# sp-uhh/audio-visual-vad

Hardware: AMD Instinct MI355X
Metric: AV frame-pairs/sec (fwd+bwd) (higher is better)
Workload: dtype f32; 1 GPU; AV_net fused training step (WaveNet-W0 encoder + ResNet-18 trunk + concat + 2xLSTM1024 + FC, masked BCE, backward, RCCL all-reduce, fused Adam): BASELINE configs[3]/[4] per-GPU shard; per_gpu_frame_pairs=1024, global_frame_pairs=1024, sequences_per_gpu=64, parallelism=dp1, reserved_cus=0, reported_block=median

## Files before the change

audio-visual-vad_amd/csrc/wavenet.hip:

```cpp
#include "gemm_api.h"
#include "wn_block.h"
#include "wn_tail.h"

namespace {

static inline int grid1(long n) { long b = (n + 255) / 256; return (int)(b > 8192 ? 8192 : (b < 1 ? 1 : b)); }

__global__ void conv1d_fwd_generic(const float* __restrict__ x, const float* __restrict__ w, const float* __restrict__ bias,
                                   const float* __restrict__ res, float* __restrict__ y, int B, int Cin, int Cout, int Lin,
                                   int Lout, int fw, int dil, int relu_in, int res_off, int res_L) {
  const long n = (long)B * Cout * Lout;
  for (long i = (long)blockIdx.x * blockDim.x + threadIdx.x; i < n; i += (long)gridDim.x * blockDim.x) {
    const int t = (int)(i % Lout);
    const int co = (int)((i / Lout) % Cout);
    const int b = (int)(i / ((long)Lout * Cout));
    float acc = bias ? bias[co] : 0.f;
    const float* xb = x + (long)b * Cin * Lin + t;
    const float* wr = w + (long)co * Cin * fw;
    for (int ci = 0; ci < Cin; ++ci)
      for (int k = 0; k < fw; ++k) {
        float v = xb[(long)ci * Lin + k * dil];
        if (relu_in) v = fmaxf(v, 0.f);
        acc = fmaf(wr[ci * fw + k], v, acc);
      }
// ... 635 lines not shown

struct DzwTile { float g[16], x[32]; };
template <bool RESIDENT>
__device__ __forceinline__ void wn_block_bwd_dz_wgrad_body(float* tiles, float* red, float* wl, float* wtl,
                                                           const float* __restrict__ dS, const float* __restrict__ w_dil,
                                                           const float* __restrict__ b_dil, const float* __restrict__ w_dense,
                                                           const float* __restrict__ s_in, float* __restrict__ DZ,
                                                           float* __restrict__ slab, int B, int Lin, int dil) {
  const int lane = threadIdx.x & 63, wave = threadIdx.x >> 6;
  const int li = lane & 31, lh = lane >> 5;
  const int Lo = Lin - dil;
  const int tiles_per_seq = tiles_per_sequence<32>(Lo);
  const int ntiles = B * tiles_per_seq;
  float* T = tiles + wave * 2 * 1056;
  float* T1 = T + 1056;
  float* Th = T + lh * 1056;
  stage_w_dil(wl, w_dil, threadIdx.x, 256);
  stage_bias(wl + WIMG_DIL_SIZE, b_dil, threadIdx.x);
  if (RESIDENT) stage_w_dense(T, w_dense, lane, 64);
  else stage_w_dense(wtl, w_dense, threadIdx.x, 256);
  for (int i = threadIdx.x; i < WG_SLAB; i += 256) red[i] = 0.f;
  __syncthreads();
  const float* wtp = (RESIDENT ? T : wtl) + lh * WIMG_DENSE_PITCH + li;
  const float* wdp = wl + li * WIMG_DIL_PITCH + lh;
  const float* bzl = wl + WIMG_DIL_SIZE + 4 * lh;
  float wt[16], wd[32];
  if (RESIDENT) {
#pragma unroll
    for (int s = 0; s < 16; ++s) wt[s] = wtp[2 * WIMG_DENSE_PITCH * s];
#pragma unroll
    for (int s = 0; s < 32; ++s) wd[s] = wdp[2 * s];
  }
  __builtin_amdgcn_wave_barrier();

  f32x16 acc0, acc1, acc2;
#pragma unroll
  for (int r = 0; r < 16; ++r) { acc0[r] = 0.f; acc1[r] = 0.f; acc2[r] = 0.f; }
  float bs_dz = 0.f, bs_ds = 0.f;
  const int rowL = Lin * 4, rowO = Lo * 4;

  auto issue = [&](int tile, DzwTile& n) __attribute__((always_inline)) {
    const TilePos p = tile_pos(tile < ntiles ? tile : ntiles - 1, tiles_per_seq, li, Lo);
    const __amdgpu_buffer_rsrc_t rg = brsrc(dS + (long)p.b * 32 * Lo, 32 * rowO);
    const __amdgpu_buffer_rsrc_t rx = brsrc(s_in + (long)p.b * 32 * Lin, 32 * rowL);
    const int offg = p.ok ? p.t * 4 + lh * rowO : BUF_OOB;
    const int offx = p.ok ? (p.t + lh * dil) * 4 : BUF_OOB;
#pragma unroll
    for (int q = 0; q < 16; ++q) n.g[q] = bload(rg, offg, 2 * q * rowO);
#pragma unroll
    for (int c = 0; c < 32; ++c) n.x[c] = bload(rx, offx, c * rowL);
  };
  auto compute = [&](int tidx, const DzwTile& c) __attribute__((always_inline)) {
    const TilePos p = tile_pos(tidx, tiles_per_seq, li, Lo);
    const int offo = p.ok ? p.t * 4 + 4 * lh * rowO : BUF_OOB;
    const __amdgpu_buffer_rsrc_t rz = brsrc(DZ + (long)p.b * 32 * Lo, 32 * rowO);
    float x[32];
#pragma unroll
    for (int s = 0; s < 32; ++s) x[s] = relu1(c.x[s]);
    f32x16 z;
#pragma unroll
    for (int r = 0; r < 16; ++r) z[r] = bzl[mfma32_row(r, 0)];
#pragma unroll
    for (int s = 0; s < 32; ++s) z = mfma32(RESIDENT ? wd[s] : wdp[2 * s], x[s], z);
    f32x16 acc;
#pragma unroll
    for (int r = 0; r < 16; ++r) acc[r] = 0.f;
#pragma unroll
    for (int q = 0; q < 16; ++q) acc = mfma32(RESIDENT ? wt[q] : wtp[2 * WIMG_DENSE_PITCH * q], c.g[q], acc);
    float f0[16], f1[16];
    __builtin_amdgcn_wave_barrier();
#pragma unroll
    for (int r = 0; r < 16; ++r) {
      const float dz = z[r] > 0.f ? acc[r] : 0.f;
      bstore(dz, rz, offo, mfma32_row(r, 0) * rowO);
      T[mfma32_row(r, lh) * 33 + li] = dz;
    }
    __builtin_amdgcn_wave_barrier();
#pragma unroll
    for (int q = 0; q < 16; ++q) { f0[q] = T[li * 33 + 2 * q + lh]; bs_dz += f0[q]; }
    __builtin_amdgcn_wave_barrier();
#pragma unroll
    for (int s = 0; s < 32; ++s) Th[s * 33 + li] = x[s];
    __builtin_amdgcn_wave_barrier();
#pragma unroll
    for (int q = 0; q < 16; ++q) f1[q] = T[li * 33 + 2 * q + lh];
#pragma unroll
    for (int q = 0; q < 16; ++q) acc0 = mfma32(f0[q], f1[q], acc0);
#pragma unroll
    for (int q = 0; q < 16; ++q) f1[q] = T1[li * 33 + 2 * q + lh];
#pragma unroll
    for (int q = 0; q < 16; ++q) acc1 = mfma32(f0[q], f1[q], acc1);
    __builtin_amdgcn_wave_barrier();
#pragma unroll
    for (int q = 0; q < 16; ++q) T[(2 * q + lh) * 33 + li] = c.g[q];
#pragma unroll
    for (int r = 0; r < 16; ++r) T1[mfma32_row(r, lh) * 33 + li] = relu1(z[r]);
    __builtin_amdgcn_wave_barrier();
#pragma unroll
    for (int q = 0; q < 16; ++q) { f0[q] = T[li * 33 + 2 * q + lh]; bs_ds += f0[q]; }
#pragma unroll
    for (int q = 0; q < 16; ++q) f1[q] = T1[li * 33 + 2 * q + lh];
#pragma unroll
    for (int q = 0; q < 16; ++q) acc2 = mfma32(f0[q], f1[q], acc2);
    __builtin_amdgcn_wave_barrier();
  };
  const TileWalkI w = xcd_walk_i(ntiles);
  DzwTile ta, tb;
  if (RESIDENT) {
    if (w.first < w.last) issue(w.first, ta);
    pingpong_tiles<true>(w, ta, tb, issue, compute);
  } else {
    plain_tiles<true, DzwTile>(w, issue, compute);
  }

  for (int wv = 0; wv < 4; ++wv) {
    __syncthreads();
    if (wave == wv) {
#pragma unroll
      for (int r = 0; r < 16; ++r) {
        const int row = mfma32_row(r, lh);
        red[row * 32 + li] += acc0[r];
        red[1024 + row * 32 + li] += acc1[r];
        red[2048 + row * 32 + li] += acc2[r];
      }
      if (lh == 0) { red[3072 + li] += bs_dz; red[3104 + li] += bs_ds; }
      __builtin_amdgcn_wave_barrier();
      if (lh == 1) { red[3072 + li] += bs_dz; red[3104 + li] += bs_ds; }
    }
  }
  __syncthreads();
  float* out = slab + (long)blockIdx.x * WG_SLAB;
  for (int i = threadIdx.x; i < WG_SLAB; i += 256) out[i] = red[i];
}

__global__ void __launch_bounds__(256)
    wn_block_bwd_dz_wgrad_mfma(const float* __restrict__ dS, const float* __restrict__ w_dil, const float* __restrict__ b_dil,
                               const float* __restrict__ w_dense, const float* __restrict__ s_in, float* __restrict__ DZ,
                               float* __restrict__ slab, int B, int Lin, int dil) {
  __shared__ float tile[4 * 2 * 32 * 33];
  __shared__ float red[WG_SLAB];
  __shared__ float wl[WIMG_DIL_SIZE + 32];
  wn_block_bwd_dz_wgrad_body<true>(tile, red, wl, nullptr, dS, w_dil, b_dil, w_dense, s_in, DZ, slab, B, Lin, dil);
}

__global__ void __launch_bounds__(256, 2)
    wn_block_bwd_dz_wgrad_occ(const float* __restrict__ dS, const float* __restrict__ w_dil, const float* __restrict__ b_dil,
                               const float* __restrict__ w_dense, const float* __restrict__ s_in, float* __restrict__ DZ,
                               float* __restrict__ slab, int B, int Lin, int dil) {
  __shared__ float tile[4 * 2 * 32 * 33];
  __shared__ float red[WG_SLAB];
  __shared__ float wl[WIMG_DIL_SIZE + 32];
  __shared__ float wtl[WIMG_DENSE_SIZE];
  wn_block_bwd_dz_wgrad_body<false>(tile, red, wl, wtl, dS, w_dil, b_dil, w_dense, s_in, DZ, slab, B, Lin, dil);
}

typedef float f4u __attribute__((ext_vector_type(4), aligned(4)));

__global__ void __launch_bounds__(256, 2)
    wn_block_bwd_dzw_t(const float* __restrict__ dS, const float* __restrict__ w_dil, const float* __restrict__ b_dil,
                       const float* __restrict__ w_dense, const float* __restrict__ s_in, float* __restrict__ DZ,
                       float* __restrict__ slab, int B, int Lin, int dil) {
  __shared__ float red[WG_SLAB];
  __shared__ float wl[WIMG_BDENSE];
  const int lane = threadIdx.x & 63;
  const int li = lane & 31, lh = lane >> 5;
  const int Lo = Lin - dil;
  const int tiles_per_seq = tiles_per_sequence<32>(Lo);
  const long ntiles = (long)B * tiles_per_seq;
  const long wave0 = ((long)blockIdx.x * blockDim.x + threadIdx.x) >> 6;
  const long nwaves = ((long)gridDim.x * blockDim.x) >> 6;
  stage_w_dil(wl + WIMG_DIL, w_dil, threadIdx.x, 256);
  stage_w_dense(wl + WIMG_DENSE, w_dense, threadIdx.x, 256);
  stage_bias(wl + WIMG_BDIL, b_dil, threadIdx.x);
  for (int i = threadIdx.x; i < WG_SLAB; i += 256) red[i] = 0.f;
  __syncthreads();
  const float* wdp = wl + WIMG_DIL + li * WIMG_DIL_PITCH + lh;
  const float* wtp = wl + WIMG_DENSE + lh * WIMG_DENSE_PITCH + li;
  const float bz = wl[WIMG_BDIL + li];

  f32x16 acc0, acc1, acc2;
#pragma unroll
  for (int r = 0; r < 16; ++r) { acc0[r] = 0.f; acc1[r] = 0.f; acc2[r] = 0.f; }
  float bs_dz = 0.f, bs_ds = 0.f;

  for (long tl = wave0; tl < ntiles; tl += nwaves) {
    const TilePos p = tile_pos(tl, tiles_per_seq, li, Lo);
    const int b = p.b, t0 = p.t0, t = p.t;
    const bool ok = p.ok;
    const int tcl = ok ? t : 0;
    const bool full = t0 + 32 <= Lo;
    float x[32], g[16];
    {
      const float* xp = s_in + (long)b * 32 * Lin + tcl + lh * dil;
#pragma unroll
      for (int c = 0; c < 32; ++c) x[c] = xp[(long)c * Lin];
      const float* gp = dS + (long)b * 32 * Lo + tcl;
#pragma unroll
      for (int q = 0; q < 16; ++q) g[q] = gp[(long)(2 * q + lh) * Lo];
    }
    float gc[16], xc0[16], xc1[16];
    const float* rowS = dS + ((long)b * 32 + li) * Lo + t0 + 4 * lh;
    const float* rowX = s_in + ((long)b * 32 + li) * Lin + t0 + 4 * lh;
    if (full) {
#pragma unroll
      for (int q = 0; q < 4; ++q) {
        const f4u a = *reinterpret_cast<const f4u*>(rowS + 8 * q);
        const f4u u = *reinterpret_cast<const f4u*>(rowX + 8 * q);
        const f4u v = *reinterpret_cast<const f4u*>(rowX + dil + 8 * q);
#pragma unroll
        for (int e = 0; e < 4; ++e) { gc[4 * q + e] = a[e]; xc0[4 * q + e] = u[e]; xc1[4 * q + e] = v[e]; }
      }
    } else {
#pragma unroll
      for (int s = 0; s < 16; ++s) {
        const int o = 8 * (s >> 2) + (s & 3);
        const bool in = t0 + 4 * lh + o < Lo;
        const int oc = in ? o : -(t0 + 4 * lh);
        const float a = rowS[oc], u = rowX[oc], v = rowX[oc + dil];
        gc[s] = in ? a : 0.f; xc0[s] = in ? u : 0.f; xc1[s] = in ? v : 0.f;
      }
    }
    __builtin_amdgcn_sched_barrier(0);
#pragma unroll
    for (int c = 0; c < 32; ++c) x[c] = ok ? relu1(x[c]) : 0.f;
#pragma unroll
    for (int q = 0; q < 16; ++q) g[q] = ok ? g[q] : 0.f;
    f32x16 zT;
#pragma unroll
    for (int r = 0; r < 16; ++r) zT[r] = bz;
#pragma unroll
    for (int s = 0; s < 32; ++s) zT = mfma32(x[s], wdp[2 * s], zT);
    f32x16 dzT;
#pragma unroll
    for (int r = 0; r < 16; ++r) dzT[r] = 0.f;
#pragma unroll
    for (int s = 0; s < 16; ++s) dzT = mfma32(g[s], wtp[66 * s], dzT);
#pragma unroll
    for (int r = 0; r < 16; ++r) dzT[r] = zT[r] > 0.f ? dzT[r] : 0.f;
    float* rowZ = DZ + ((long)b * 32 + li) * Lo + t0 + 4 * lh;
    if (full) {
#pragma unroll
      for (int q = 0; q < 4; ++q) {
        f4u o = {dzT[4 * q], dzT[4 * q + 1], dzT[4 * q + 2], dzT[4 * q + 3]};
        *reinterpret_cast<f4u*>(rowZ + 8 * q) = o;
      }
    } else {
#pragma unroll
      for (int s = 0; s < 16; ++s) {
        const int o = 8 * (s >> 2) + (s & 3);
        if (t0 + 4 * lh + o < Lo) rowZ[o] = dzT[s];
      }
    }
#pragma unroll
    for (int s = 0; s < 16; ++s) { bs_dz += dzT[s]; bs_ds += gc[s]; }
#pragma unroll
    for (int s = 0; s < 16; ++s) acc2 = mfma32(gc[s], relu1(zT[s]), acc2);
#pragma unroll
    for (int s = 0; s < 16; ++s) acc0 = mfma32(dzT[s], relu1(xc0[s]), acc0);
#pragma unroll
    for (int s = 0; s < 16; ++s) acc1 = mfma32(dzT[s], relu1(xc1[s]), acc1);
  }

#pragma unroll
  for (int r = 0; r < 16; ++r) {
    const int row = mfma32_row(r, lh);
    atomicAdd(&red[row * 32 + li], acc0[r]);
    atomicAdd(&red[1024 + row * 32 + li], acc1[r]);
    atomicAdd(&red[2048 + row * 32 + li], acc2[r]);
  }
  atomicAdd(&red[3072 + li], bs_dz);
  atomicAdd(&red[3104 + li], bs_ds);
  __syncthreads();
  float* out = slab + (long)blockIdx.x * WG_SLAB;
  for (int i = threadIdx.x; i < WG_SLAB; i += 256) out[i] = red[i];
}

constexpr int WN_MAXL = 64;
struct WgradTab {
  const float* slab[WN_MAXL];
  int nslab[WN_MAXL];
  float* dW_dil[WN_MAXL];
  float* db_dil[WN_MAXL];
  float* dW_dense[WN_MAXL];
  float* db_dense[WN_MAXL];
};
__global__ void __launch_bounds__(256) wn_wgrad_reduce_all(const WgradTab tab) {
  const int l = blockIdx.y;
  const int i = blockIdx.x * 32 + (threadIdx.x & 31);
  const int nslab = tab.nslab[l];
  const float s = slab_sum_fixed_order(tab.slab[l] + i, nslab, WG_SLAB);
  if (threadIdx.x >= 32 || nslab <= 0) return;
  if (i < 2048) { if (tab.dW_dil[l]) tab.dW_dil[l][(i & 1023) * 2 + (i >> 10)] += s; }
  else if (i < 3072) { if (tab.dW_dense[l]) tab.dW_dense[l][i - 2048] += s; }
  else if (i < 3104) { if (tab.db_dil[l]) tab.db_dil[l][i - 3072] += s; }
  else if (tab.db_dense[l]) tab.db_dense[l][i - 3104] += s;
}

struct Plan {
  int n;
  int L[66];
  size_t s[66];
  size_t z, dz, ga, gb, dzt;
  size_t zs[66];
  size_t slab;
  size_t gslab;
  size_t total;
};
static int make_plan(const avvad_wavenet_desc* d, Plan* p) {
  if (!d || d->n_layers < 0 || d->n_layers > 64 || d->B <= 0 || d->fw < 1 || d->qc < 1 || d->R < 1 || d->D < 1 ||
      d->Bn < 1 || d->P < 1 || (d->n_layers > 0 && !d->dilations_h))
    return AVVAD_EINVAL;
  p->n = d->n_layers;
  p->L[0] = d->L - (d->fw - 1);
  for (int i = 0; i < p->n; ++i) p->L[i + 1] = p->L[i] - d->dilations_h[i] * (d->fw - 1);
  if (p->L[p->n] < 1) return AVVAD_EINVAL;
  size_t off = 0;
  auto take = [&](size_t n) { size_t o = off; off += align_up(n, 64); return o; };
  const size_t B = d->B;
  if (d->save_for_backward) {
    for (int i = 0; i <= p->n; ++i) p->s[i] = take(B * d->R * p->L[i]);
    const size_t big = B * (size_t)(d->R > d->D ? d->R : d->D) * p->L[0];
    p->z = take(big); p->dz = take(big); p->ga = take(big); p->gb = take(big);
    p->dzt = take(B * d->Bn * p->L[p->n]);
    {
      const size_t zb = (d->R == 32 && d->D == 32 && d->fw == 2 && p->n > 0) ? take(B * d->D * p->L[1]) : 0;
      for (int i = 0; i < p->n; ++i) p->zs[i] = zb;
    }
    {
      const bool perlayer = d->R == 32 && d->D == 32 && d->fw == 2;
      const size_t a = (size_t)WG_MAXBLK * WG_SLAB * (perlayer ? (size_t)p->n : 1), b2 = (size_t)TAIL_MAXBLK * tail_slab_floats(d->Bn);
      p->slab = take(a > b2 ? a : b2);
    }
    p->gslab = take(igemm::SLAB_FLOATS);
  } else {
    for (int i = 0; i < p->n; ++i) p->zs[i] = 0;
    const size_t a = take(B * d->R * p->L[0]), b2 = take(B * d->R * p->L[0]);
    for (int i = 0; i <= p->n; ++i) p->s[i] = (i & 1) ? b2 : a;
    p->z = take(B * d->D * p->L[0]);
    p->dz = p->ga = p->gb = p->dzt = 0;
  }
  p->total = off;
  return AVVAD_OK;
}

static inline bool mfma_shape(const avvad_wavenet_desc* d) { return d->R == 32 && d->D == 32 && d->fw == 2; }
static inline bool buf_ok(int B, int Lin) {
  return avvad_tune().wn_flat != 1 && (long)Lin * 32 * 4 + 4096 < (1L << 31) && (long)B * cdiv(Lin, 32) < (1L << 31);
}

enum class FwdForm { FLAT, BUF, OCC, WIDE, DMA };
enum class DxForm { FLAT, BUF, OCC };
enum class BwdForm { RESIDENT, OCC, TRANSPOSED, UNFUSED };
enum class TailFwdForm { GENERIC, MFMA1, MFMA4 };
enum class TailBwdForm { PAIR, FUSED, MFMA, GENERIC };
struct FwdChoice { FwdForm form; int grid; };
struct DxChoice { DxForm form; int grid; };
struct BwdChoice { BwdForm form; int grid; int grid_z, grid_dz; };
struct TailFwdChoice { TailFwdForm form; int grid; };
struct TailBwdChoice { TailBwdForm form; int grid; };

enum class XcdRound { NONE, UP, UP_FROM_8, DOWN_FROM_8 };
static int wn_grid_size(long tiles, int per_wg, long cap, int wn_grid, XcdRound r) {
  long g = (tiles + per_wg - 1) / per_wg;
  if (g > cap) g = cap;
  if (wn_grid > 0 && g > wn_grid) g = wn_grid;
  if (r == XcdRound::UP || (r == XcdRound::UP_FROM_8 && g >= 8)) g = (g + 7) / 8 * 8;
  if (r == XcdRound::DOWN_FROM_8 && g >= 8) g = g / 8 * 8;
  return (int)(g < 1 ? 1 : g);
}

constexpr int WIDE_FROM = 8192;
static FwdChoice fwd_form(int B, int Lin, int dil) {
  const AvvadTune& t = avvad_tune();
  const int Lo = Lin - dil;
  const bool buf = buf_ok(B, Lin);
  if (buf && (t.wn_flat == 0 || t.wn_flat == 3) && Lo >= 128 && (Lo >= WIDE_FROM || t.wn_flat == 3))
    return {FwdForm::WIDE, wn_grid_size((long)B * cdiv(Lo, 128), 4, t.wn_grid > 0 ? t.wn_grid : 1024, 0, XcdRound::UP)};
  const long ntiles = (long)B * cdiv(Lo, 32);
  if (buf && t.wn_flat == 5 && Lo >= 32)
    return {FwdForm::DMA, wn_grid_size(ntiles, 8, 512, t.wn_grid, XcdRound::UP_FROM_8)};
  if (buf && (t.wn_flat == 0 || t.wn_flat == 4))
    return {FwdForm::OCC, wn_grid_size(ntiles, 4, 1024, t.wn_grid, XcdRound::UP_FROM_8)};
  return {buf ? FwdForm::BUF : FwdForm::FLAT, wn_grid_size(ntiles, 4, 512, t.wn_grid, XcdRound::NONE)};
}

static DxChoice dx_form(int B, int Lin) {
  const AvvadTune& t = avvad_tune();
  const long ntiles = (long)B * cdiv(Lin, 32);
  if (buf_ok(B, Lin) && (t.wn_dx == 0 || t.wn_dx == 2))
    return {DxForm::OCC, wn_grid_size(ntiles, 4, 1024, 0, XcdRound::UP_FROM_8)};
  return {buf_ok(B, Lin) && t.wn_dx != 3 ? DxForm::BUF : DxForm::FLAT, wn_grid_size(ntiles, 4, 512, 0, XcdRound::NONE)};
}

static BwdChoice bwd_form(int B, int Lo, bool shared_device, bool any_grad) {
  const AvvadTune& t = avvad_tune();
  const long ntiles = (long)B * cdiv(Lo, 32);
  if (!any_grad || t.wn_no_fused_wgrad)
    return {BwdForm::UNFUSED, wn_grid_size(ntiles, 16, WG_MAXBLK, 0, XcdRound::NONE), wn_grid_size(ntiles, 4, 512, 0, XcdRound::NONE),
            wn_grid_size(ntiles, 4, 768, 0, XcdRound::NONE)};
  switch (t.wn_bwd_t == 0 ? (shared_device ? 3 : 2) : t.wn_bwd_t) {
    case 3:
      return {BwdForm::RESIDENT, wn_grid_size(ntiles, 16, 256, 0, XcdRound::NONE), 0, 0};
    case 2:
      return {BwdForm::OCC, wn_grid_size(ntiles, 16, WG_MAXBLK, 0, XcdRound::DOWN_FROM_8), 0, 0};
    default:
      return {BwdForm::TRANSPOSED, wn_grid_size(ntiles, 16, WG_MAXBLK, 0, XcdRound::NONE), 0, 0};
  }
}

static TailFwdChoice tail_fwd_form(int B, int R, int Bn, int P) {
  if (!(R == 32 && Bn % 32 == 0)) return {TailFwdForm::GENERIC, 0};
  const int nt = Bn % 128 == 0 ? 4 : 1;
  return {nt == 4 ? TailFwdForm::MFMA4 : TailFwdForm::MFMA1, wn_grid_size((long)B * P * (Bn / (32 * nt)), 4, 2048, 0, XcdRound::NONE)};
}

static TailBwdChoice tail_bwd_form(int B, int Lv, int R, int Bn, int P, bool any_grad) {
  const AvvadTune& t = avvad_tune();
  const long ntiles = (long)B * cdiv(Lv, 32);
  if (!(R == 32 && Bn % 32 == 0 && Bn <= 1024) || P > Lv) return {TailBwdForm::GENERIC, 0};
  if (Bn == 256 && any_grad && !t.wn_no_fused_tail)
    return {t.wn_no_tail_pair ? TailBwdForm::FUSED : TailBwdForm::PAIR, wn_grid_size(ntiles, 4, TAIL_MAXBLK, 0, XcdRound::NONE)};
  return {TailBwdForm::MFMA, wn_grid_size(ntiles, 4, 2048, 0, XcdRound::NONE)};
}

static void launch_block_fwd(const float* s_in, const float* wd, const float* bd, const float* we, const float* be, float* s_out,
                             int B, int Lin, int dil, hipStream_t s) {
  const FwdChoice c = fwd_form(B, Lin, dil);
  const dim3 grid(c.grid);
  switch (c.form) {
    case FwdForm::WIDE: hipLaunchKernelGGL(wn_block_fwd_w4, grid, dim3(256), 0, s, s_in, wd, bd, we, be, s_out, B, Lin, dil); break;
    case FwdForm::DMA: hipLaunchKernelGGL(wn_block_fwd_dma, grid, dim3(512), 0, s, s_in, wd, bd, we, be, s_out, B, Lin, dil); break;
    case FwdForm::OCC: hipLaunchKernelGGL(wn_block_fwd_occ, grid, dim3(256), 0, s, s_in, wd, bd, we, be, s_out, B, Lin, dil); break;
    case FwdForm::BUF: hipLaunchKernelGGL(wn_block_fwd_buf, grid, dim3(256), 0, s, s_in, wd, bd, we, be, s_out, B, Lin, dil); break;
    case FwdForm::FLAT:
      hipLaunchKernelGGL(wn_block_fwd_mfma<0>, grid, dim3(256), 0, s, s_in, wd, bd, we, be, s_out, (float*)nullptr, B, Lin, dil);
      break;
  }
}

static int wgrad_conv1d(const float* dy, const float* x, float* dw, int B, int Cout, int Cin, int Lout, int Lin, int fw,
                        int dil, int relu_in, hipStream_t s, float* slab) {
  const long K = (long)B * Lout;
  if (K > 0x7fffffffL) return AVVAD_EINVAL;
  const int ktiles = cdiv(K, igemm::BK);
  int split = 1024 / (cdiv(Cout, 64) * cdiv(Cin * fw, 64));
  if (split > ktiles) split = ktiles;
  if (split < 1) split = 1;
  igemm::RowSegK a{dy, Lout, (long)Cout * Lout, Cout, (int)K, Lout, 0, 0, 1, 0};
  igemm::RowSegK b{x, Lin, (long)Cin * Lin, Cin * fw, (int)K, Lout, 0, relu_in, fw, dil};
  igemm::EpiStore e{dw, (long)Cin * fw, nullptr, 1};
  return igemm::launch<64, 64>(a, b, e, Cout, Cin * fw, (int)K, split, s, slab);
}

static void bias_grad(const float* dy, float* db, int B, int C, int L, hipStream_t s) {
  if (!db) return;
  hipLaunchKernelGGL(chan_sum_acc, dim3(C, 1), dim3(256), 0, s, dy, db, B, C, L);
}

static void launch_tail_fwd(const float* sN, const float* wb, const float* bb, float* out, int B, int R, int Bn, int Lv, int P,
                            hipStream_t s) {
  const TailFwdChoice c = tail_fwd_form(B, R, Bn, P);
  switch (c.form) {
    case TailFwdForm::MFMA4: hipLaunchKernelGGL(tail_fwd_mfma<4>, dim3(c.grid), dim3(256), 0, s, sN, wb, bb, out, B, Bn, Lv, P); break;
    case TailFwdForm::MFMA1: hipLaunchKernelGGL(tail_fwd_mfma<1>, dim3(c.grid), dim3(256), 0, s, sN, wb, bb, out, B, Bn, Lv, P); break;
    case TailFwdForm::GENERIC: hipLaunchKernelGGL(tail_fwd_generic, dim3(P, B), dim3(256), 0, s, sN, wb, bb, out, R, Bn, Lv, P); break;
  }
}

static int launch_tail_bwd(const float* sN, const float* wb, const float* bb, const float* dout, float* dW, float* db, float* dS,
                           float* dzt, float* slab, float* gslab, int B, int R, int Bn, int Lv, int P, hipStream_t s) {
  const TailBwdChoice c = tail_bwd_form(B, Lv, R, Bn, P, dW || db);
  int rc;
  if (c.form == TailBwdForm::PAIR || c.form == TailBwdForm::FUSED) {
    const bool pair = c.form == TailBwdForm::PAIR;
    const size_t lds = (size_t)tail_fused_lds_floats(Bn, pair ? 2 : 1) * sizeof(float);
    if ((rc = pair ? allow_large_lds<tail_bwd_wgrad_pair<8>>(lds, lds) : allow_large_lds<tail_bwd_wgrad_mfma<8>>(lds, lds))) return rc;
    hipLaunchKernelGGL(pair ? tail_bwd_wgrad_pair<8> : tail_bwd_wgrad_mfma<8>, dim3(c.grid), dim3(pair ? 512 : 256), lds, s, sN, wb,
                       bb, dout, dS, slab, B, Lv, P);
    hipLaunchKernelGGL(tail_wgrad_reduce, dim3(cdiv(tail_slab_floats(Bn), 32)), dim3(256), 0, s, slab, c.grid, Bn, dW, db);
    return AVVAD_OK;
  }
  if (c.form == TailBwdForm::MFMA)
    hipLaunchKernelGGL(tail_bwd_mfma, dim3(c.grid), dim3(256), (size_t)tail_wimg_floats(Bn) * sizeof(float), s, sN, wb, bb, dout,
                       dzt, dS, B, Bn, Lv, P);
  else
    hipLaunchKernelGGL(tail_bwd_dz_generic, dim3(grid1((long)B * Bn * Lv)), dim3(256), 0, s, sN, wb, bb, dout, dzt, B, R, Bn, Lv, P);
  if (dW && (rc = wgrad_conv1d(dzt, sN, dW, B, Bn, R, Lv, Lv, 1, 1, 0, s, gslab))) return rc;
  bias_grad(dzt, db, B, Bn, Lv, s);
  if (c.form == TailBwdForm::GENERIC)
    hipLaunchKernelGGL(conv1d_bwd_data_generic, dim3(grid1((long)B * R * Lv)), dim3(256), 0, s, dzt, wb, (const float*)nullptr,
                       (const float*)nullptr, dS, B, R, Bn, Lv, Lv, 1, 1, 0, 0);
  return AVVAD_OK;
}

}

extern "C" size_t avvad_wavenet_workspace(const avvad_wavenet_desc* d) {
  Plan p;
  if (make_plan(d, &p)) return 0;
  return p.total * sizeof(float);
}

extern "C" int avvad_wavenet_fwd(const float* wave, const avvad_wavenet_params* prm, float* out, const avvad_wavenet_desc* d,
                                 void* wsv, size_t ws_bytes, avvad_stream_t sv) {
  AVVAD_ENTER();
  Plan p;
  if (!wave || !prm || !out || !wsv || ws_misaligned(wsv) || make_plan(d, &p)) return AVVAD_EINVAL;
  if (ws_bytes < p.total * sizeof(float)) return AVVAD_EWORKSPACE;
  hipStream_t s = (hipStream_t)sv;
  float* ws = (float*)wsv;
  const int B = d->B, R = d->R, D = d->D, fw = d->fw;
  hipLaunchKernelGGL(conv1d_fwd_generic, dim3(grid1((long)B * R * p.L[0])), dim3(256), 0, s, wave, prm->causal_w,
                     d->use_bias ? prm->causal_b : (const float*)nullptr, (const float*)nullptr, ws + p.s[0], B, d->qc, R,
                     d->L, p.L[0], fw, 1, 0, 0, 0);
  for (int i = 0; i < p.n; ++i) {
    const int dil = d->dilations_h[i];
    const float* bd = d->use_bias ? prm->dil_b_h[i] : nullptr;
    const float* be = d->use_bias ? prm->dense_b_h[i] : nullptr;
    if (mfma_shape(d)) {
      launch_block_fwd(ws + p.s[i], prm->dil_w_h[i], bd, prm->dense_w_h[i], be, ws + p.s[i + 1], B, p.L[i], dil, s);
    } else {
      float* z = ws + p.z;
      hipLaunchKernelGGL(conv1d_fwd_generic, dim3(grid1((long)B * D * p.L[i + 1])), dim3(256), 0, s, ws + p.s[i],
                         prm->dil_w_h[i], bd, (const float*)nullptr, z, B, R, D, p.L[i], p.L[i + 1], fw, dil, 1, 0, 0);
      hipLaunchKernelGGL(conv1d_fwd_generic, dim3(grid1((long)B * R * p.L[i + 1])), dim3(256), 0, s, z, prm->dense_w_h[i], be,
                         ws + p.s[i], ws + p.s[i + 1], B, D, R, p.L[i + 1], p.L[i + 1], 1, 1, 1, p.L[i] - p.L[i + 1], p.L[i]);
    }
  }
  launch_tail_fwd(ws + p.s[p.n], prm->bott_w, d->use_bias ? prm->bott_b : (const float*)nullptr, out, B, R, d->Bn, p.L[p.n],
                  d->P, s);
  AVVAD_LAUNCH_CHECK();
  return AVVAD_OK;
}

extern "C" int avvad_wavenet_block_fwd(const float* s_in, const float* w_dil, const float* b_dil, const float* w_dense,
                                       const float* b_dense, float* s_out, int B, int Lin, int dil, avvad_stream_t sv) {
  AVVAD_ENTER();
  if (!s_in || !w_dil || !w_dense || !s_out || B <= 0 || dil < 1 || Lin - dil < 1) return AVVAD_EINVAL;
  launch_block_fwd(s_in, w_dil, b_dil, w_dense, b_dense, s_out, B, Lin, dil, (hipStream_t)sv);
  AVVAD_LAUNCH_CHECK();
  return AVVAD_OK;
}

extern "C" int avvad_wavenet_bwd(const float* wave, const avvad_wavenet_params* prm, const float* dout,
                                 const avvad_wavenet_grads* g, float* dwave, const avvad_wavenet_desc* d, void* wsv,
                                 size_t ws_bytes, avvad_stream_t sv) {
  AVVAD_ENTER();
  Plan p;
  if (!wave || !prm || !dout || !g || !wsv || ws_misaligned(wsv) || make_plan(d, &p) || !d->save_for_backward) return AVVAD_EINVAL;
  if (ws_bytes < p.total * sizeof(float)) return AVVAD_EWORKSPACE;
  hipStream_t s = (hipStream_t)sv;
  float* ws = (float*)wsv;
  const int B = d->B, R = d->R, D = d->D, fw = d->fw, Bn = d->Bn;
  int rc;
  float* Z = ws + p.z;
  float* DZ = ws + p.dz;
  float* GA = ws + p.ga;
  float* GB = ws + p.gb;
  if ((rc = launch_tail_bwd(ws + p.s[p.n], prm->bott_w, d->use_bias ? prm->bott_b : (const float*)nullptr, dout, g->bott_w,
                            d->use_bias ? g->bott_b : (float*)nullptr, GA, ws + p.dzt, ws + p.slab, ws + p.gslab, B, R, Bn,
                            p.L[p.n], d->P, s)))
    return rc;
  WgradTab wtab;
  bool any_slab = false;
  for (int l = 0; l < WN_MAXL; ++l) {
    wtab.slab[l] = nullptr; wtab.nslab[l] = 0;
    wtab.dW_dil[l] = wtab.db_dil[l] = wtab.dW_dense[l] = wtab.db_dense[l] = nullptr;
  }
  auto note_slabs = [&](int i, float* slab_i, int wb) {
    wtab.slab[i] = slab_i; wtab.nslab[i] = wb;
    wtab.dW_dil[i] = g->dil_w_h[i]; wtab.dW_dense[i] = g->dense_w_h[i];
    wtab.db_dil[i] = d->use_bias ? g->dil_b_h[i] : (float*)nullptr;
    wtab.db_dense[i] = d->use_bias ? g->dense_b_h[i] : (float*)nullptr;
    any_slab = true;
  };
  for (int i = p.n - 1; i >= 0; --i) {
    float* const slab_i = ws + p.slab + (size_t)i * WG_MAXBLK * WG_SLAB;
    const int dil = d->dilations_h[i];
    const int Li = p.L[i], Lo = p.L[i + 1];
    const float* si = ws + p.s[i];
    const float* bd = d->use_bias ? prm->dil_b_h[i] : nullptr;
    const bool fast = mfma_shape(d);
    float* Zi = fast ? ws + p.zs[i] : Z;
    if (!fast)
      hipLaunchKernelGGL(conv1d_fwd_generic, dim3(grid1((long)B * D * Lo)), dim3(256), 0, s, si, prm->dil_w_h[i], bd,
                         (const float*)nullptr, Zi, B, R, D, Li, Lo, fw, dil, 1, 0, 0);
    if (fast) {
      const bool any_grad = g->dil_w_h[i] || g->dense_w_h[i] || (d->use_bias && (g->dil_b_h[i] || g->dense_b_h[i]));
      const BwdChoice bc = bwd_form(B, Lo, d->shared_device != 0, any_grad);
      switch (bc.form) {
        case BwdForm::RESIDENT:
          hipLaunchKernelGGL(wn_block_bwd_dz_wgrad_mfma, dim3(bc.grid), dim3(256), 0, s, GA, prm->dil_w_h[i], bd,
                             prm->dense_w_h[i], si, DZ, slab_i, B, Li, dil);
          break;
        case BwdForm::OCC:
          hipLaunchKernelGGL(wn_block_bwd_dz_wgrad_occ, dim3(bc.grid), dim3(256), 0, s, GA, prm->dil_w_h[i], bd,
                             prm->dense_w_h[i], si, DZ, slab_i, B, Li, dil);
          break;
        case BwdForm::TRANSPOSED:
          hipLaunchKernelGGL(wn_block_bwd_dzw_t, dim3(bc.grid), dim3(256), 0, s, GA, prm->dil_w_h[i], bd, prm->dense_w_h[i], si,
                             DZ, slab_i, B, Li, dil);
          break;
        case BwdForm::UNFUSED:
          hipLaunchKernelGGL(wn_block_fwd_mfma<2>, dim3(bc.grid_z), dim3(256), 0, s, si, prm->dil_w_h[i], bd, prm->dense_w_h[i],
                             (const float*)nullptr, (float*)nullptr, Zi, B, Li, dil);
          hipLaunchKernelGGL(wn_block_bwd_dz_mfma, dim3(bc.grid_dz), dim3(256), 0, s, GA, Zi, prm->dense_w_h[i], DZ, B, Lo);
          if (any_grad)
            hipLaunchKernelGGL(wn_block_wgrad_mfma, dim3(bc.grid), dim3(256), 0, s, GA, Zi, DZ, si, slab_i, B, Li, dil);
          break;
      }
      if (any_grad) note_slabs(i, slab_i, bc.grid);
      const DxChoice dc = dx_form(B, Li);
      switch (dc.form) {
        case DxForm::OCC:
          hipLaunchKernelGGL(wn_block_bwd_dx_occ, dim3(dc.grid), dim3(256), 0, s, DZ, si, GA, prm->dil_w_h[i], GB, B, Li, dil);
          break;
        case DxForm::BUF:
          hipLaunchKernelGGL(wn_block_bwd_dx_buf, dim3(dc.grid), dim3(256), 0, s, DZ, si, GA, prm->dil_w_h[i], GB, B, Li, dil);
          break;
        case DxForm::FLAT:
          hipLaunchKernelGGL(wn_block_bwd_dx_mfma, dim3(dc.grid), dim3(256), 0, s, DZ, si, GA, prm->dil_w_h[i], GB, B, Li, dil);
          break;
      }
    } else {
      if (g->dense_w_h[i] && (rc = wgrad_conv1d(GA, Zi, g->dense_w_h[i], B, R, D, Lo, Lo, 1, 1, 1, s, ws + p.gslab))) return rc;
      if (d->use_bias) bias_grad(GA, g->dense_b_h[i], B, R, Lo, s);
      hipLaunchKernelGGL(conv1d_bwd_data_generic, dim3(grid1((long)B * D * Lo)), dim3(256), 0, s, GA, prm->dense_w_h[i], Zi,
                         (const float*)nullptr, DZ, B, D, R, Lo, Lo, 1, 1, 0, 0);
      if (g->dil_w_h[i] && (rc = wgrad_conv1d(DZ, si, g->dil_w_h[i], B, D, R, Lo, Li, fw, dil, 1, s, ws + p.gslab))) return rc;
      if (d->use_bias) bias_grad(DZ, g->dil_b_h[i], B, D, Lo, s);
      hipLaunchKernelGGL(conv1d_bwd_data_generic, dim3(grid1((long)B * R * Li)), dim3(256), 0, s, DZ, prm->dil_w_h[i], si, GA,
                         GB, B, R, D, Li, Lo, fw, dil, Li - Lo, Lo);
    }
    float* t = GA; GA = GB; GB = t;
  }
  if (any_slab) hipLaunchKernelGGL(wn_wgrad_reduce_all, dim3(WG_SLAB / 32, p.n), dim3(256), 0, s, wtab);
  if (d->qc * fw <= 4) {
    if (g->causal_w || (d->use_bias && g->causal_b))
    {
      const int ny = B < 32 ? B : 32;
      float* part = ws + p.gslab;
      hipLaunchKernelGGL(narrow_conv1d_grads, dim3(R, ny), dim3(256), 0, s, GA, wave, part, B, R, d->qc, p.L[0], d->L, fw);
      hipLaunchKernelGGL(narrow_conv1d_grads_sum, dim3(cdiv(R * 5, 256)), dim3(256), 0, s, part, ny, R, d->qc * fw, g->causal_w,
                         d->use_bias ? g->causal_b : (float*)nullptr);
    }
  } else {
    if (g->causal_w && (rc = wgrad_conv1d(GA, wave, g->causal_w, B, R, d->qc, p.L[0], d->L, fw, 1, 0, s, ws + p.gslab))) return rc;
    if (d->use_bias) bias_grad(GA, g->causal_b, B, R, p.L[0], s);
  }
  if (dwave)
    hipLaunchKernelGGL(conv1d_bwd_data_generic, dim3(grid1((long)B * d->qc * d->L)), dim3(256), 0, s, GA, prm->causal_w,
                       (const float*)nullptr, (const float*)nullptr, dwave, B, d->qc, R, d->L, p.L[0], fw, 1, 0, 0);
  AVVAD_LAUNCH_CHECK();
  return AVVAD_OK;
}
```

audio-visual-vad_amd/csrc/wn_block.h:

```cpp
#pragma once
#include "common.h"

constexpr int WIMG_DIL_PITCH = 65, WIMG_DENSE_PITCH = 33;
constexpr int WIMG_DIL = 0;
constexpr int WIMG_DENSE = WIMG_DIL + 32 * WIMG_DIL_PITCH;
constexpr int WIMG_BDIL = WIMG_DENSE + 32 * WIMG_DENSE_PITCH;
constexpr int WIMG_BDENSE = WIMG_BDIL + 32;
constexpr int WIMG_SIZE = WIMG_BDENSE + 32;
constexpr int WIMG_DIL_SIZE = WIMG_DENSE;
constexpr int WIMG_DENSE_SIZE = 32 * WIMG_DENSE_PITCH;

__device__ __forceinline__ void stage_w_dil(float* img, const float* __restrict__ w_dil, int tid, int nthreads) {
  for (int i = tid; i < 2048; i += nthreads) img[(i >> 6) * WIMG_DIL_PITCH + (i & 63)] = w_dil[i];
}
__device__ __forceinline__ void stage_w_dense(float* img, const float* __restrict__ w_dense, int tid, int nthreads) {
  for (int i = tid; i < 1024; i += nthreads) img[(i >> 5) * WIMG_DENSE_PITCH + (i & 31)] = w_dense[i];
}
__device__ __forceinline__ void stage_bias(float* img, const float* __restrict__ b, int tid) {
  if (tid < 32) img[tid] = b ? b[tid] : 0.f;
}
__device__ __forceinline__ void stage_block_weights(float* img, const float* __restrict__ w_dil, const float* __restrict__ b_dil,
                                                    const float* __restrict__ w_dense, const float* __restrict__ b_dense,
                                                    int tid, int nthreads) {
  stage_w_dil(img + WIMG_DIL, w_dil, tid, nthreads);
  stage_w_dense(img + WIMG_DENSE, w_dense, tid, nthreads);
  stage_bias(img + WIMG_BDIL, b_dil, tid);
  stage_bias(img + WIMG_BDENSE, b_dense, tid);
}

template <int W>
__device__ __forceinline__ int tiles_per_sequence(int L) { return (L + W - 1) >> __builtin_ctz(W); }
struct TilePos { int b, t0, t; bool ok; };
template <int W = 32, class I>
__device__ __forceinline__ TilePos tile_pos(I tile, int tiles_per_seq, int lane_off, int L) {
  TilePos p;
  p.b = (int)(tile / tiles_per_seq);
  p.t0 = (int)(tile - (I)p.b * tiles_per_seq) * W;
  p.t = p.t0 + lane_off;
  p.ok = p.t < L;
  return p;
}

template <bool PIN, class Set, class Issue, class Compute>
__device__ __forceinline__ void pingpong_tiles(const TileWalkI& w, Set& a, Set& b, Issue issue, Compute compute) {
  for (int tile = w.first; tile < w.last; tile += 2 * w.stride) {
    issue(tile + w.stride, b);
    if (PIN) __builtin_amdgcn_sched_barrier(0);
    compute(tile, a);
    if (tile + w.stride >= w.last) break;
    issue(tile + 2 * w.stride, a);
    if (PIN) __builtin_amdgcn_sched_barrier(0);
    compute(tile + w.stride, b);
  }
}
template <bool PIN, class Set, class Issue, class Compute>
__device__ __forceinline__ void plain_tiles(const TileWalkI& w, Issue issue, Compute compute) {
  for (int tile = w.first; tile < w.last; tile += w.stride) {
    Set a;
    issue(tile, a);
    if (PIN) __builtin_amdgcn_sched_barrier(0);
    compute(tile, a);
  }
}
```

Before: 60670 frame-pairs/s.

## Fuse WaveNet block backward dz, wgrad and dx into one chained-segment kernel

Adds a new backward kernel that walks each sequence in dilation-strided chains of 32-wide tiles and keeps the previous tile's dz in LDS. This lets it compute the dz, the weight-gradient accumulation and the dx/residual output in a single pass, and it becomes the default backward form, so the separate dx kernel launch and the DZ round trip through global memory are skipped. The cost is a much larger dynamic LDS footprint, more per-wave register state, and sequential dependency within chains that can limit parallelism. Small sequence counts may also leave segments unevenly balanced.

```diff
diff --git a/audio-visual-vad_amd/csrc/wavenet.hip b/audio-visual-vad_amd/csrc/wavenet.hip
--- a/audio-visual-vad_amd/csrc/wavenet.hip
+++ b/audio-visual-vad_amd/csrc/wavenet.hip
@@ -811,6 +811,203 @@
   __shared__ float wl[WIMG_DIL_SIZE + 32];
   __shared__ float wtl[WIMG_DENSE_SIZE];
   wn_block_bwd_dz_wgrad_body<false>(tile, red, wl, wtl, dS, w_dil, b_dil, w_dense, s_in, DZ, slab, B, Lin, dil);
+}
+
+constexpr int BLK_TILES = 4 * 3 * 1056;
+constexpr int BLK_LDS_FLOATS = BLK_TILES + WG_SLAB + WIMG_DIL_SIZE + 32 + WIMG_DENSE_SIZE;
+struct BlkTile { float g[16], x[32], rv[16]; };
+template <bool RESIDENT>
+__device__ __forceinline__ void wn_block_bwd_block_body(float* blk_lds, const float* __restrict__ dS, const float* __restrict__ w_dil,
+                                                        const float* __restrict__ b_dil, const float* __restrict__ w_dense,
+                                                        const float* __restrict__ s_in, float* __restrict__ dS_in,
+                                                        float* __restrict__ slab, int B, int Lin, int dil, int S) {
+  float* const red = blk_lds + BLK_TILES;
+  float* const wl = red + WG_SLAB;
+  float* const wtl = wl + WIMG_DIL_SIZE + 32;
+  const int lane = threadIdx.x & 63, wave = threadIdx.x >> 6;
+  const int li = lane & 31, lh = lane >> 5;
+  const int Lo = Lin - dil;
+  const ChainPlan cp = chain_plan(Lin, dil, S);
+  const int nseg = (int)chain_segments(cp, B);
+  float* cur = blk_lds + wave * 3 * 1056;
+  float* prev = cur + 1056;
+  float* const T1 = cur + 2 * 1056;
+  stage_w_dil(wl, w_dil, threadIdx.x, 256);
+  stage_bias(wl + WIMG_DIL_SIZE, b_dil, threadIdx.x);
+  stage_w_dense(wtl, w_dense, threadIdx.x, 256);
+  for (int i = threadIdx.x; i < WG_SLAB; i += 256) red[i] = 0.f;
+  __syncthreads();
+  const float* wtp = wtl + lh * WIMG_DENSE_PITCH + li;
+  const float* wdp = wl + li * WIMG_DIL_PITCH + lh;
+  const float* wxp = wl + li * 2 + lh;
+  const float* bzl = wl + WIMG_DIL_SIZE + 4 * lh;
+  const int col = li - (dil < 32 ? dil : 32);
+  float wt[16], wd[32], wx[32];
+  if (RESIDENT) {
+#pragma unroll
+    for (int s = 0; s < 16; ++s) wt[s] = wtp[2 * WIMG_DENSE_PITCH * s];
+#pragma unroll
+    for (int s = 0; s < 32; ++s) { wd[s] = wdp[2 * s]; wx[s] = wxp[WIMG_DIL_PITCH * s]; }
+  }
+
+  f32x16 acc0, acc1, acc2;
+#pragma unroll
+  for (int r = 0; r < 16; ++r) { acc0[r] = 0.f; acc1[r] = 0.f; acc2[r] = 0.f; }
+  float bs_dz = 0.f, bs_ds = 0.f;
+  const int rowL = Lin * 4, rowO = Lo * 4;
+
+  const TileWalkI w = xcd_walk_i(nseg);
+  for (int sg = w.first; sg < w.last; sg += w.stride) {
+    const ChainSeg seg = chain_seg(cp, sg);
+    if (seg.n == 0) continue;
+    const __amdgpu_buffer_rsrc_t rg = brsrc(dS + (long)seg.b * 32 * Lo, 32 * rowO);
+    const __amdgpu_buffer_rsrc_t rx = brsrc(s_in + (long)seg.b * 32 * Lin, 32 * rowL);
+    const __amdgpu_buffer_rsrc_t ro = brsrc(dS_in + (long)seg.b * 32 * Lin, 32 * rowL);
+    auto issue = [&](int i, BlkTile& n) __attribute__((always_inline)) {
+      const int t = (seg.u0 + i * cp.k) * 32 + li;
+      const bool on = i < seg.n;
+      const int offg = on && t < Lo ? t * 4 + lh * rowO : BUF_OOB;
+      const int offx = on && t + lh * dil < Lin ? (t + lh * dil) * 4 : BUF_OOB;
+      const int offr = on && i >= 0 && t >= dil && t < Lin ? (t - dil) * 4 + 4 * lh * rowO : BUF_OOB;
+#pragma unroll
+      for (int q = 0; q < 16; ++q) n.g[q] = bload(rg, offg, 2 * q * rowO);
+#pragma unroll
+      for (int s = 0; s < 32; ++s) n.x[s] = bload(rx, offx, s * rowL);
+#pragma unroll
+      for (int r = 0; r < 16; ++r) n.rv[r] = bload(rg, offr, mfma32_row(r, 0) * rowO);
+    };
+    auto compute = [&](int i, const BlkTile& c) __attribute__((always_inline)) {
+      const bool live = i >= 0;
+      const int t = (seg.u0 + i * cp.k) * 32 + li;
+      float x[32];
+#pragma unroll
+      for (int s = 0; s < 32; ++s) x[s] = relu1(c.x[s]);
+      f32x16 z;
+#pragma unroll
+      for (int r = 0; r < 16; ++r) z[r] = bzl[mfma32_row(r, 0)];
+#pragma unroll
+      for (int s = 0; s < 32; ++s) z = mfma32(RESIDENT ? wd[s] : wdp[2 * s], x[s], z);
+      f32x16 acc;
+#pragma unroll
+      for (int r = 0; r < 16; ++r) acc[r] = 0.f;
+#pragma unroll
+      for (int q = 0; q < 16; ++q) acc = mfma32(RESIDENT ? wt[q] : wtp[2 * WIMG_DENSE_PITCH * q], c.g[q], acc);
+      __builtin_amdgcn_wave_barrier();
+#pragma unroll
+      for (int r = 0; r < 16; ++r) cur[mfma32_row(r, lh) * 33 + li] = z[r] > 0.f ? acc[r] : 0.f;
+      __builtin_amdgcn_wave_barrier();
+      if (live) {
+        float f0[16], f1[16];
+        const float* bsrc = lh == 0 ? cur + li : (col >= 0 ? cur + col : prev + col + 32);
+        f32x16 ax;
+        {
+          float bz[32];
+#pragma unroll
+          for (int s = 0; s < 32; ++s) bz[s] = bsrc[s * 33];
+          __builtin_amdgcn_wave_barrier();
+#pragma unroll
+          for (int r = 0; r < 16; ++r) ax[r] = 0.f;
+#pragma unroll
+          for (int s = 0; s < 32; ++s) ax = mfma32(RESIDENT ? wx[s] : wxp[WIMG_DIL_PITCH * s], bz[s], ax);
+        }
+#pragma unroll
+        for (int q = 0; q < 16; ++q) { f0[q] = cur[li * 33 + 2 * q + lh]; bs_dz += f0[q]; }
+        float* Th = lh == 0 ? prev : T1;
+#pragma unroll
+        for (int s = 0; s < 32; ++s) Th[s * 33 + li] = x[s];
+        __builtin_amdgcn_wave_barrier();
+#pragma unroll
+        for (int q = 0; q < 16; ++q) f1[q] = prev[li * 33 + 2 * q + lh];
+#pragma unroll
+        for (int q = 0; q < 16; ++q) acc0 = mfma32(f0[q], f1[q], acc0);
+#pragma unroll
+        for (int q = 0; q < 16; ++q) f1[q] = T1[li * 33 + 2 * q + lh];
+#pragma unroll
+        for (int q = 0; q < 16; ++q) acc1 = mfma32(f0[q], f1[q], acc1);
+        {
+          const int offo = t < Lin ? t * 4 + 4 * lh * rowL : BUF_OOB;
+#pragma unroll
+          for (int r = 0; r < 16; ++r) {
+            const float m = prev[mfma32_row(r, lh) * 33 + li];
+            bstore((m > 0.f ? ax[r] : 0.f) + c.rv[r], ro, offo, mfma32_row(r, 0) * rowL);
+          }
+        }
+        __builtin_amdgcn_wave_barrier();
+#pragma unroll
+        for (int q = 0; q < 16; ++q) prev[(2 * q + lh) * 33 + li] = c.g[q];
+#pragma unroll
+        for (int r = 0; r < 16; ++r) T1[mfma32_row(r, lh) * 33 + li] = relu1(z[r]);
+        __builtin_amdgcn_wave_barrier();
+#pragma unroll
+        for (int q = 0; q < 16; ++q) { f0[q] = prev[li * 33 + 2 * q + lh]; bs_ds += f0[q]; }
+#pragma unroll
+        for (int q = 0; q < 16; ++q) f1[q] = T1[li * 33 + 2 * q + lh];
+#pragma unroll
+        for (int q = 0; q < 16; ++q) acc2 = mfma32(f0[q], f1[q], acc2);
+        __builtin_amdgcn_wave_barrier();
+      }
+      float* const sw = cur; cur = prev; prev = sw;
+    };
+    const int i0 = seg.head ? -1 : 0;
+    BlkTile ta, tb;
+    if (RESIDENT) issue(i0, ta);
+    if (!seg.head) {
+      __builtin_amdgcn_wave_barrier();
+      for (int i = lane; i < 1056; i += 64) prev[i] = 0.f;
+    }
+    if (RESIDENT) {
+      for (int i = i0; i < seg.n; i += 2) {
+        issue(i + 1, tb);
+        __builtin_amdgcn_sched_barrier(0);
+        compute(i, ta);
+        if (i + 1 >= seg.n) break;
+        issue(i + 2, ta);
+        __builtin_amdgcn_sched_barrier(0);
+        compute(i + 1, tb);
+      }
+    } else {
+      for (int i = i0; i < seg.n; ++i) {
+        issue(i, ta);
+        __builtin_amdgcn_sched_barrier(0);
+        compute(i, ta);
+      }
+    }
+  }
+
+  for (int wv = 0; wv < 4; ++wv) {
+    __syncthreads();
+    if (wave == wv) {
+#pragma unroll
+      for (int r = 0; r < 16; ++r) {
+        const int row = mfma32_row(r, lh);
+        red[row * 32 + li] += acc0[r];
+        red[1024 + row * 32 + li] += acc1[r];
+        red[2048 + row * 32 + li] += acc2[r];
+      }
+      if (lh == 0) { red[3072 + li] += bs_dz; red[3104 + li] += bs_ds; }
+      __builtin_amdgcn_wave_barrier();
+      if (lh == 1) { red[3072 + li] += bs_dz; red[3104 + li] += bs_ds; }
+    }
+  }
+  __syncthreads();
+  float* out = slab + (long)blockIdx.x * WG_SLAB;
+  for (int i = threadIdx.x; i < WG_SLAB; i += 256) out[i] = red[i];
+}
+
+__global__ void __launch_bounds__(256, 2)
+    wn_block_bwd_block(const float* __restrict__ dS, const float* __restrict__ w_dil, const float* __restrict__ b_dil,
+                       const float* __restrict__ w_dense, const float* __restrict__ s_in, float* __restrict__ dS_in,
+                       float* __restrict__ slab, int B, int Lin, int dil, int S) {
+  extern __shared__ float blk_lds[];
+  wn_block_bwd_block_body<false>(blk_lds, dS, w_dil, b_dil, w_dense, s_in, dS_in, slab, B, Lin, dil, S);
+}
+
+__global__ void __launch_bounds__(256)
+    wn_block_bwd_block_res(const float* __restrict__ dS, const float* __restrict__ w_dil, const float* __restrict__ b_dil,
+                           const float* __restrict__ w_dense, const float* __restrict__ s_in, float* __restrict__ dS_in,
+                           float* __restrict__ slab, int B, int Lin, int dil, int S) {
+  extern __shared__ float blk_lds[];
+  wn_block_bwd_block_body<true>(blk_lds, dS, w_dil, b_dil, w_dense, s_in, dS_in, slab, B, Lin, dil, S);
 }
 
 typedef float f4u __attribute__((ext_vector_type(4), aligned(4)));
@@ -1009,12 +1206,12 @@
 
 enum class FwdForm { FLAT, BUF, OCC, WIDE, DMA };
 enum class DxForm { FLAT, BUF, OCC };
-enum class BwdForm { RESIDENT, OCC, TRANSPOSED, UNFUSED };
+enum class BwdForm { RESIDENT, OCC, TRANSPOSED, UNFUSED, BLOCK, BLOCK_RESIDENT };
 enum class TailFwdForm { GENERIC, MFMA1, MFMA4 };
 enum class TailBwdForm { PAIR, FUSED, MFMA, GENERIC };
 struct FwdChoice { FwdForm form; int grid; };
 struct DxChoice { DxForm form; int grid; };
-struct BwdChoice { BwdForm form; int grid; int grid_z, grid_dz; };
+struct BwdChoice { BwdForm form; int grid; int grid_z, grid_dz; int seg; };
 struct TailFwdChoice { TailFwdForm form; int grid; };
 struct TailBwdChoice { TailBwdForm form; int grid; };
 
@@ -1051,13 +1248,25 @@
   return {buf_ok(B, Lin) && t.wn_dx != 3 ? DxForm::BUF : DxForm::FLAT, wn_grid_size(ntiles, 4, 512, 0, XcdRound::NONE)};
 }
 
-static BwdChoice bwd_form(int B, int Lo, bool shared_device, bool any_grad) {
+constexpr int BLK_SEG_MIN = 4;
+static BwdChoice bwd_form(int B, int Lo, int dil, bool shared_device, bool any_grad) {
   const AvvadTune& t = avvad_tune();
   const long ntiles = (long)B * cdiv(Lo, 32);
   if (!any_grad || t.wn_no_fused_wgrad)
     return {BwdForm::UNFUSED, wn_grid_size(ntiles, 16, WG_MAXBLK, 0, XcdRound::NONE), wn_grid_size(ntiles, 4, 512, 0, XcdRound::NONE),
             wn_grid_size(ntiles, 4, 768, 0, XcdRound::NONE)};
-  switch (t.wn_bwd_t == 0 ? (shared_device ? 3 : 2) : t.wn_bwd_t) {
+  int form = t.wn_bwd_t == 0 ? (shared_device ? 5 : 4) : t.wn_bwd_t;
+  if (form == 4 || form == 5) {
+    const int Lin = Lo + dil;
+    const long tiles_in = (long)B * cdiv(Lin, 32);
+    const int grid = wn_grid_size(tiles_in, 16, form == 5 ? 256 : WG_MAXBLK, 0, XcdRound::DOWN_FROM_8);
+    const int per_wave = cdiv(tiles_in, 4L * grid);
+    const int seg = per_wave > BLK_SEG_MIN ? per_wave : BLK_SEG_MIN;
+    if ((dil % 32 == 0 || dil < 32) && buf_ok(B, Lin) && chain_segments(chain_plan(Lin, dil, seg), B) < (1L << 31))
+      return {form == 5 ? BwdForm::BLOCK_RESIDENT : BwdForm::BLOCK, grid, 0, 0, seg};
+    form -= 2;
+  }
+  switch (form) {
     case 3:
       return {BwdForm::RESIDENT, wn_grid_size(ntiles, 16, 256, 0, XcdRound::NONE), 0, 0};
     case 2:
@@ -1246,8 +1455,17 @@
                          (const float*)nullptr, Zi, B, R, D, Li, Lo, fw, dil, 1, 0, 0);
     if (fast) {
       const bool any_grad = g->dil_w_h[i] || g->dense_w_h[i] || (d->use_bias && (g->dil_b_h[i] || g->dense_b_h[i]));
-      const BwdChoice bc = bwd_form(B, Lo, d->shared_device != 0, any_grad);
+      const BwdChoice bc = bwd_form(B, Lo, dil, d->shared_device != 0, any_grad);
       switch (bc.form) {
+        case BwdForm::BLOCK:
+        case BwdForm::BLOCK_RESIDENT: {
+          const bool res = bc.form == BwdForm::BLOCK_RESIDENT;
+          const size_t lds = (size_t)BLK_LDS_FLOATS * sizeof(float);
+          if ((rc = res ? allow_large_lds<wn_block_bwd_block_res>(lds, lds) : allow_large_lds<wn_block_bwd_block>(lds, lds))) return rc;
+          hipLaunchKernelGGL(res ? wn_block_bwd_block_res : wn_block_bwd_block, dim3(bc.grid), dim3(256), lds, s, GA, prm->dil_w_h[i],
+                             bd, prm->dense_w_h[i], si, GB, slab_i, B, Li, dil, bc.seg);
+          break;
+        }
         case BwdForm::RESIDENT:
           hipLaunchKernelGGL(wn_block_bwd_dz_wgrad_mfma, dim3(bc.grid), dim3(256), 0, s, GA, prm->dil_w_h[i], bd,
                              prm->dense_w_h[i], si, DZ, slab_i, B, Li, dil);
@@ -1270,7 +1488,7 @@
       }
       if (any_grad) note_slabs(i, slab_i, bc.grid);
       const DxChoice dc = dx_form(B, Li);
-      switch (dc.form) {
+      if (bc.form != BwdForm::BLOCK && bc.form != BwdForm::BLOCK_RESIDENT) switch (dc.form) {
         case DxForm::OCC:
           hipLaunchKernelGGL(wn_block_bwd_dx_occ, dim3(dc.grid), dim3(256), 0, s, DZ, si, GA, prm->dil_w_h[i], GB, B, Li, dil);
           break;
diff --git a/audio-visual-vad_amd/csrc/wn_block.h b/audio-visual-vad_amd/csrc/wn_block.h
--- a/audio-visual-vad_amd/csrc/wn_block.h
+++ b/audio-visual-vad_amd/csrc/wn_block.h
@@ -41,6 +41,29 @@
   return p;
 }
 
+struct ChainPlan { int k, S, tiles, per_chain; };
+__device__ __host__ __forceinline__ ChainPlan chain_plan(int Lin, int dil, int S) {
+  ChainPlan c;
+  c.k = dil >= 32 ? dil >> 5 : 1;
+  c.S = S;
+  c.tiles = (Lin + 31) >> 5;
+  c.per_chain = ((c.tiles + c.k - 1) / c.k + S - 1) / S;
+  return c;
+}
+__device__ __host__ __forceinline__ long chain_segments(const ChainPlan& c, int B) { return (long)B * c.k * c.per_chain; }
+struct ChainSeg { int b, u0, n; bool head; };
+__device__ __forceinline__ ChainSeg chain_seg(const ChainPlan& c, int sg) {
+  const int per_seq = c.k * c.per_chain;
+  ChainSeg s;
+  s.b = sg / per_seq;
+  const int r = sg - s.b * per_seq, j = r / c.k;
+  s.u0 = (r - j * c.k) + j * c.S * c.k;
+  const int left = s.u0 < c.tiles ? (c.tiles - s.u0 + c.k - 1) / c.k : 0;
+  s.n = left < c.S ? left : c.S;
+  s.head = j > 0;
+  return s;
+}
+
 template <bool PIN, class Set, class Issue, class Compute>
 __device__ __forceinline__ void pingpong_tiles(const TileWalkI& w, Set& a, Set& b, Issue issue, Compute compute) {
   for (int tile = w.first; tile < w.last; tile += 2 * w.stride) {
```

Measured after the change: 61150 frame-pairs/s (median of 6 runs). Within noise of the previous version (+0.8%).
